# nichmorgan/better-search-rag-rust

Hardware: AMD Instinct MI355X
Metric: queries/sec + p50 latency, 768-d top-10 over N vectors @1/2/4/8 GPU (higher is better)
Workload: dtype f32; 1 GPU; configs[2]: 10M x 768 f32 corpus sharded over the N GPUs, 1000 batched queries, top-10; rows_total=10000000, rows_per_gpu_rank0=10000000, queries=1000, top_k=10, dim=768, parallelism=corpus sharded over 1 GPU(s) (interval_by_rank)

## Files before the change

better-search-rag-rust_amd/csrc/index.cpp:

```cpp
#include <math.h>
#include <stdio.h>
#include <string.h>

#include <algorithm>

#include "internal.hpp"
#include "kernels.hpp"

namespace bsr {

constexpr uint32_t kMaxKForFilter = 200;

static thread_local std::string g_err;

int set_error(int code, const char* fmt, ...) {
    char buf[1024];
    va_list ap;
    va_start(ap, fmt);
    vsnprintf(buf, sizeof buf, fmt, ap);
    va_end(ap);
    g_err = buf;
    return code;
}
void clear_error() { g_err.clear(); }
// ... 325 lines not shown
    if (nq > kSkinnyMaxQ || ix->n < kSkinnyTopMinRows || kp_for(k) > 63 || k > 64 || ix->op_row_bytes > 16 * 64 ||
        ix->ld % 64 != 0 || ix->ld > 1024 || !rescore_kp_enabled())
        return 0;
    const uint32_t slots = 4 * skinny_top_lists((uint32_t)ix->n);
    return slots <= 64u * kTopKeysPerLane ? slots : 0;
}

static int filter_buffers(bsr_index* ix, uint32_t nq, uint32_t qpad, uint32_t k, uint32_t cap_in = 0) {
    const uint32_t kp = kp_for(k);
    const uint32_t cap = std::max(cap_in ? cap_in : cap_for(k), top_slots(ix, nq, k));
    ix->stats.n_candidates = kp;
    BSR_TRY(ix->tau.ensure((size_t)qpad * sizeof(float)));
    BSR_TRY(ix->cand.ensure((size_t)qpad * cap * sizeof(uint64_t)));
    BSR_TRY(ix->cnt.ensure(((size_t)qpad + 8 * kTailCounters + kGangWords) * sizeof(uint32_t)));
    BSR_TRY(ix->cand_rows.ensure((size_t)nq * kp * sizeof(uint32_t)));
    BSR_TRY(ix->ncand.ensure((size_t)nq * sizeof(uint32_t)));
    BSR_TRY(ix->tau_excl.ensure((size_t)nq * sizeof(float)));
    BSR_TRY(ix->fail.ensure((size_t)nq * sizeof(uint32_t)));
    BSR_TRY(ix->fail2.ensure((size_t)nq * sizeof(uint32_t)));
    return BSR_OK;
}

static GemmArgs gemm_args(bsr_index* ix, uint32_t qpad) {
    GemmArgs g{};
    g.A = ix->fop.as<uint8_t>();
    g.B = ix->qop.as<uint8_t>();
    g.row_bytes = ix->op_row_bytes;
    g.n_qt = qpad / kFilterTile;
    g.a_scale = ix->ascale.as<float>();
    g.b_scale = ix->qscale.as<float>();
    return g;
}

static int sample_pass(bsr_index* ix, uint32_t nq, uint32_t qpad, uint32_t k, uint64_t* smax, uint32_t ks_in,
                       uint32_t cap_in) {
    BSR_TRY(filter_buffers(ix, nq, qpad, k, cap_in));
    const bool skinny = nq <= kSkinnyMaxQ;
    const uint32_t cap = cap_in ? cap_in : cap_for(k);
    const uint32_t ks = ks_in ? ks_in : ks_for(k);
    const uint32_t BM = kFilterTile;
    const uint64_t n = ix->n;
    GemmArgs g = gemm_args(ix, qpad);
    uint32_t* status = ix->d_status;
    if (n > cap) {
        const uint32_t n_s = (uint32_t)((n + kSampleStride - 1) / kSampleStride);
        const uint32_t n_rt_s = (n_s + BM - 1) / BM;
        const bool compact = n_s >= 32u * 8u * ks;
        const uint32_t s_ld = compact ? n_rt_s * (BM / 32) : n_rt_s * BM;
        const uint32_t n_vals = compact ? (n_s + 31) / 32 : n_s;
        BSR_TRY(ix->S.ensure((size_t)qpad * s_ld * sizeof(float)));
        g.A = ix->fop_s.as<uint8_t>();
        g.a_stride = ix->op_row_bytes;
        g.a_scale = ix->ascale_s.as<float>();
        g.a_scale_rows = kSampleScaleRows;
        g.n_rows = n_s;
        g.n_rt = n_rt_s;
        g.S = ix->S.as<float>();
        g.s_ld = s_ld;
        g.s_compact = compact ? 1u : 0u;
        BSR_HIP(launch_timed(ix, ix->ev_sample, [&](hipEvent_t e0, hipEvent_t e1) {
            return skinny ? launch_filter_skinny_sample(g, ix->stream, e0, e1)
                          : launch_filter_sample(g, ix->stream, e0, e1);
        }, 2));
        BSR_HIP(launch_select_tau(ix->S.as<float>(), s_ld, n_vals, nq, qpad, ix->qflags.as<uint32_t>(), ks,
                                  ix->tau.as<float>(), ix->cnt.as<uint32_t>(), status, ix->stream, smax));
    } else {
        BSR_HIP(launch_select_tau(nullptr, 0, 0, nq, qpad, ix->qflags.as<uint32_t>(), ks, ix->tau.as<float>(),
                                  ix->cnt.as<uint32_t>(), status, ix->stream, smax));
    }
    return BSR_OK;
}

static int emit_pass(bsr_index* ix, uint32_t nq, uint32_t qpad, uint32_t k, uint32_t cap_in) {
    const bool skinny = nq <= kSkinnyMaxQ;
    const uint32_t BM = kFilterTile;
    const uint64_t n = ix->n;
    GemmArgs g = gemm_args(ix, qpad);
    g.a_stride = ix->op_row_bytes;
    g.a_scale_rows = kQuantBlock;
    g.n_rows = (uint32_t)n;
    g.n_rt = (uint32_t)((n + BM - 1) / BM);
    g.tau = ix->tau.as<float>();
    g.cand = ix->cand.as<uint64_t>();
    g.cnt = ix->cnt.as<uint32_t>();
    g.cap = cap_in ? cap_in : cap_for(k);
    g.tail = g.n_qt <= kTailCounters ? ix->cnt.as<uint32_t>() + qpad : nullptr;
    BSR_HIP(launch_timed(ix, ix->ev_emit, [&](hipEvent_t e0, hipEvent_t e1) {
        return skinny ? launch_filter_skinny_emit(g, ix->stream, e0, e1)
                      : launch_filter_emit(g, ix->stream, e0, e1);
    }));
    return BSR_OK;
}

static uint32_t top_layout_lab() {
    const char* lay = getenv("BSR_TOP_LAYOUT");
    return lay && lay[0] == '0' ? 0u : 2u;
}

static int top_pass(bsr_index* ix, uint32_t nq, uint32_t qpad, uint32_t k) {
    BSR_TRY(filter_buffers(ix, nq, qpad, k));
    GemmArgs g = gemm_args(ix, qpad);
    g.a_stride = ix->op_row_bytes;
    g.a_scale_rows = kQuantBlock;
    g.n_rows = (uint32_t)ix->n;
    g.n_rt = (uint32_t)((ix->n + kFilterTile - 1) / kFilterTile);
    g.cand = ix->cand.as<uint64_t>();
    g.cnt = ix->cnt.as<uint32_t>();
    g.cap = top_slots(ix, nq, k);
    g.status = ix->d_status;
    g.n_q = nq;
    g.top_layout = top_layout_lab();
    BSR_HIP(launch_timed(ix, ix->ev_emit, [&](hipEvent_t e0, hipEvent_t e1) {
        return launch_filter_skinny_top(g, ix->stream, e0, e1);
    }));
    return BSR_OK;
}

static int run_filter(bsr_index* ix, uint32_t nq, uint32_t qpad, uint32_t k, uint32_t* next_status, bool publish) {
    const uint32_t top = top_slots(ix, nq, k);
    if (top) {
        BSR_TRY(top_pass(ix, nq, qpad, k));
    } else {
// ... 170 lines not shown
    qa.qf32 = qf32.as<float>();
    qa.nb = nb.as<float>();
    qa.qop = qop.p;
    qa.qscale = qscale.as<float>();
    qa.ebound = ebound.as<float>();
    qa.qflags = qflags.as<uint32_t>();
    qa.qids = qids_id.as<int32_t>();
    qa.status = d_status;
    qa.with_op = use_filter;
    const bool publish = use_filter && n > 0 && (!profiling(ix) || prof_level <= 1);
    auto enqueue_search = [&]() -> int {
        BSR_HIP(launch_query_prep(qa, stream));
        if (n == 0) {
            BSR_HIP(hipMemsetAsync(keys.p, 0xff, (size_t)nq * k * sizeof(uint64_t), stream));
        } else if (!use_filter) {
            stats.n_exact_direct = nq;
            BSR_TRY(run_exact_scan(ix, qids_id.as<int32_t>(), nq, k));
        } else {
            BSR_TRY(run_filter(ix, nq, qpad, k, next_status, publish));
        }
        if (!(use_filter && n > 0))
            BSR_HIP(launch_finalize(keys.as<uint64_t>(), nq, k, n, global_offset, d_idx, d_dist, d_cnt, next_status,
                                    nullptr, d_status, stream));
        ev_end(ix, ev_total);
        if (!publish) BSR_HIP(hipMemcpyAsync(h_res, res[cur].p, res_bytes, hipMemcpyDeviceToHost, stream));
        return BSR_OK;
    };
    if (publish) __atomic_store_n(h_flag, 0u, __ATOMIC_RELEASE);

    const bool top = use_filter && top_slots(ix, nq, k) != 0;
    if (top) stats.search_path |= BSR_PATH_SKINNY_TOP;
    const bool graphable = use_filter && n > 0 && (!profiling(ix) || prof_level == 0) && !force_threshold;
    SearchGraph& gs = graphs[cur];
    const uint32_t lay = (top ? top_layout_lab() : 2u) | (skinny_glds_on() ? 0x100u : 0u);
    const bool same_shape = warm.nq == nq && warm.k == k && warm.qsrc == qsrc && warm.n == n &&
                            warm.timed == (profiling(ix) ? prof_level : 0) && warm.top == top &&
                            warm.top_layout == lay;
    const int timed_level = profiling(ix) ? prof_level : 0;
    if (graphable && gs.exec && gs.nq == nq && gs.k == k && gs.qsrc == qsrc && gs.n == n && gs.gen == g_alloc_gen &&
        gs.timed == timed_level && gs.top == top && gs.top_layout == lay) {
        BSR_HIP(hipGraphLaunch(gs.exec, stream));
        stats.n_candidates = kp_for(k);
        ++graph_replays;
        stats.graph_replay = 1;
    } else if (graphable && same_shape && warm.gen == g_alloc_gen) {
        if (gs.exec) { (void)hipGraphExecDestroy(gs.exec); gs.exec = nullptr; }
        BSR_HIP(hipStreamBeginCapture(stream, hipStreamCaptureModeThreadLocal));
        const uint64_t gen0 = g_alloc_gen;
        capturing = true;
        const int rc = enqueue_search();
        capturing = false;
        hipGraph_t graph = nullptr;
        const hipError_t ec = hipStreamEndCapture(stream, &graph);
        if (rc != BSR_OK) { if (graph) (void)hipGraphDestroy(graph); return rc; }
        if (ec != hipSuccess || g_alloc_gen != gen0) {
            if (graph) (void)hipGraphDestroy(graph);
            return set_error(BSR_E_HIP, "search graph capture failed: %s", hipGetErrorString(ec));
        }
        hipGraphExec_t exec = nullptr;
        const hipError_t ei = hipGraphInstantiate(&exec, graph, nullptr, nullptr, 0);
        (void)hipGraphDestroy(graph);
        if (ei != hipSuccess) return set_error(BSR_E_HIP, "hipGraphInstantiate: %s", hipGetErrorString(ei));
        gs = SearchGraph{exec, nq, k, qsrc, n, g_alloc_gen, timed_level, top, lay};
        BSR_HIP(hipGraphLaunch(gs.exec, stream));
        ++graph_replays;
        stats.graph_replay = 1;
    } else {
// ... 288 lines not shown
        stats.search_path |= BSR_PATH_MASK_LIST;
        BSR_TRY(build_list());
        BSR_TRY(run_list_scan(ix, qids.as<int32_t>(), nfail, k, A));
        BSR_TRY(finalize_and_read());
    }
    return BSR_OK;
}

bool bsr_index::gtau_eligible(uint32_t nq, uint32_t k) const {
    return loaded && nq > 0 && k >= 1 && k <= cfg.max_k && k <= kMaxKForFilter && approx_ok && n > cap_for(k);
}

int bsr_index::gtau_prepare(const float* queries, uint32_t nq, uint32_t k) {
    if (!gtau_eligible(nq, k)) return set_error(BSR_E_STATE, "global-threshold search not applicable");
    if (!queries) return set_error(BSR_E_INVALID, "null queries");
    BSR_HIP(hipSetDevice(device));
    stats = bsr_search_stats{};
    stats.n_queries = nq;
    stats.row_ebound = row_ebound;
    BSR_TRY(prepare_result(nq, k));
    const uint32_t qpad = (uint32_t)round_up(nq, kFilterTile);
    const uint32_t ks = ks_for(k);
    BSR_TRY(qf32.ensure((size_t)qpad * ld * sizeof(float)));
    BSR_TRY(nb.ensure((size_t)qpad * sizeof(float)));
    BSR_TRY(qop.ensure((size_t)qpad * op_row_bytes));
    BSR_TRY(qscale.ensure((size_t)qpad * sizeof(float)));
    BSR_TRY(ebound.ensure((size_t)qpad * sizeof(float)));
    BSR_TRY(qflags.ensure((size_t)qpad * sizeof(uint32_t)));
    BSR_TRY(qids_id.ensure((size_t)qpad * sizeof(int32_t)));
    BSR_TRY(keys.ensure((size_t)nq * k * sizeof(uint64_t)));
    BSR_TRY(smax.ensure((size_t)qpad * ks * sizeof(uint64_t)));
    if (!is_device_ptr(queries)) BSR_TRY(q_in.ensure((size_t)nq * dim * sizeof(float)));
    BSR_TRY(filter_buffers(this, nq, qpad, k));
    const uint32_t n_s = (uint32_t)((n + kSampleStride - 1) / kSampleStride);
    const uint32_t n_rt_s = (n_s + kFilterTile - 1) / kFilterTile;
    const bool compact = n_s >= 32u * 8u * ks;
    const uint32_t s_ld = compact ? n_rt_s * (kFilterTile / 32) : n_rt_s * kFilterTile;
    BSR_TRY(S.ensure((size_t)qpad * s_ld * sizeof(float)));
    gt_nq = nq;
    gt_k = k;
    gt_qpad = qpad;
    gt_ks = ks;
    return BSR_OK;
}

int bsr_index::gtau_phase_a(const float* queries, int part) {
    bsr_index* ix = this;
    const uint32_t nq = gt_nq, k = gt_k, qpad = gt_qpad;
    if (part == 1) {
        BSR_TRY(sample_pass(ix, nq, qpad, k, smax.as<uint64_t>()));
        return BSR_OK;
    }
    const float* qsrc = queries;
    if (!is_device_ptr(queries)) {
        BSR_HIP(hipMemcpyAsync(q_in.p, queries, (size_t)nq * dim * sizeof(float), hipMemcpyHostToDevice, stream));
        qsrc = q_in.as<float>();
    }
    ev_begin(ix, ev_total);
    QueryPrepArgs qa{};
    qa.q = qsrc;
    qa.nq = nq;
    qa.qpad = qpad;
    qa.dim = dim;
    qa.ld = ld;
    qa.ea_max = flags.as<uint32_t>() + 1;
    qa.qf32 = qf32.as<float>();
    qa.nb = nb.as<float>();
    qa.qop = qop.p;
    qa.qscale = qscale.as<float>();
    qa.ebound = ebound.as<float>();
    qa.qflags = qflags.as<uint32_t>();
// ... 105 lines not shown
```

better-search-rag-rust_amd/csrc/internal.hpp:

```cpp
#pragma once

#include <hip/hip_runtime.h>
#include <stdarg.h>
#include <stdint.h>

#include <atomic>

#include <string>
#include <vector>

#include "bsr.h"
#include "kernels.hpp"

namespace bsr {

int set_error(int code, const char* fmt, ...);
void clear_error();

#define BSR_HIP(call)                                                                       \
    do {                                                                                    \
        hipError_t e_ = (call);                                                             \
        if (e_ != hipSuccess)                                                               \
            return ::bsr::set_error(BSR_E_HIP, "%s failed: %s (%s:%d)", #call,              \
                                    hipGetErrorString(e_), __FILE__, __LINE__);             \
// ... 20 lines not shown
void* coherent_host_alias(const void* p);
hipError_t stream_wait(hipStream_t s);
hipError_t flag_wait(const uint32_t* flag, hipStream_t s);
int select_device(int device);

static inline uint64_t round_up(uint64_t x, uint64_t m) { return (x + m - 1) / m * m; }

struct Events {
    hipEvent_t a = nullptr, b = nullptr;
    bool armed = false;
    ~Events();
    int create();
};

}

struct bsr_index {
    bsr_config cfg{};
    int device = 0;
    hipStream_t stream = nullptr;
    uint32_t dim = 0, ld = 0;
    uint64_t n = 0, n_pad = 0, global_offset = 0;
    bool loaded = false;
    bool approx_ok = false;
    uint32_t row_flags = 0;
    uint32_t op_row_bytes = 0;
    float row_ebound = 0.0f;

    bsr::DevBuf rows;
    bsr::DevBuf na;
    bsr::DevBuf fop;
    bsr::DevBuf fop_s;
    bsr::DevBuf ascale_s;
    bsr::DevBuf ascale;
    bsr::DevBuf flags;

    bsr::DevBuf q_in, qf32, nb, qop, qscale, ebound, qflags, tau, S, cand, cnt, cand_rows, ncand,
        tau_excl, keys, fail, fail2, part, qids, qids_id, tmp;

    bsr::DevBuf res[2];
    uint8_t* h_res = nullptr;
    uint8_t* h_res_dev = nullptr;
    size_t h_res_bytes = 0;
    uint32_t* h_flag = nullptr;
    uint32_t* h_flag_dev = nullptr;
    bsr::DevBuf pub_ticket;
    uint32_t cur = 0;
    bool next_status_clean = false;
    size_t res_off_cnt = 0, res_off_dist = 0, res_off_idx = 0, res_off_x = 0, res_bytes = 0;
    uint32_t* d_status = nullptr;
    uint32_t* d_cnt = nullptr;
    float* d_dist = nullptr;
    uint64_t* d_idx = nullptr;
    float* d_x = nullptr;

    std::vector<uint32_t> h_qflags, h_fail;

    bsr_search_stats stats{};
    bsr_profile prof{};
    bsr::Events ev_emit, ev_sample, ev_select, ev_rescore, ev_scan, ev_total;
    int prof_level = 2;

    struct SearchGraph {
        hipGraphExec_t exec = nullptr;
        uint32_t nq = 0, k = 0;
        const float* qsrc = nullptr;
// ... 31 lines not shown
```

better-search-rag-rust_amd/csrc/k_filter.hip:

```cpp
#include <cstdlib>
#include "bsr_device.hpp"
#include "kernels.hpp"

#include <hip/hip_ext.h>

#include <math.h>

#include <algorithm>
#include <type_traits>
#include <utility>

namespace bsr {

typedef __attribute__((ext_vector_type(4))) int i32x4_t;
typedef __attribute__((ext_vector_type(16))) int i32x16_t;
typedef __attribute__((address_space(3))) void lds_void_t;

struct OpI8 {
    using frag_t = i32x4_t;
    using acc_t = i32x16_t;
    static constexpr bool kInt = true;
    __device__ __forceinline__ static acc_t mfma(const frag_t& a, const frag_t& b, const acc_t& c) {
        return __builtin_amdgcn_mfma_i32_32x32x32_i8(a, b, c, 0, 0, 0);
    }
};

constexpr int kSlots = 4;
constexpr int kSliceB = 64;
constexpr int kWCap = 256;
constexpr int kThreads = 512;

__device__ __forceinline__ void wait_vm0() { asm volatile("s_waitcnt vmcnt(0)" ::: "memory"); }

template <int N>
__device__ __forceinline__ void mid_barrier() {
    if constexpr (N == 8) asm volatile("s_waitcnt vmcnt(8) lgkmcnt(0)\n\ts_barrier" ::: "memory");
    else if constexpr (N == 6) asm volatile("s_waitcnt vmcnt(6) lgkmcnt(0)\n\ts_barrier" ::: "memory");
    else if constexpr (N == 4) asm volatile("s_waitcnt vmcnt(4) lgkmcnt(0)\n\ts_barrier" ::: "memory");
// ... 375 lines not shown
    do {                                                                                \
        __builtin_amdgcn_sched_barrier(0);                                              \
        asm volatile("s_memtime %0\n\ts_waitcnt lgkmcnt(0)" : "=s"(V_)::"memory");       \
        __builtin_amdgcn_sched_barrier(0);                                              \
    } while (0)
#endif
template <bool EMIT, int NK, int EPI = 0, int TAILX = 8, int GANG = 2, int RING = 0, int L2 = 0, int FW = 1,
          int KSB = 0>
__global__ __launch_bounds__(512, 1) void k_filter_qs16(GemmArgs p) {
    constexpr bool DEFER = EPI == 1, STAGE = EPI == 2 && EMIT;
    constexpr bool SPLIT = EPI == 3 && EMIT;
    constexpr int S = RING ? 12 : 8, A = RING == 1 ? 9 : RING == 2 ? 10 : 6;
    constexpr int kWaitN = A - 4, kYoung = A - 4, kClaimUse = ((A - 4) % 2 == 0 ? A - 3 : A - 2) + 1;
    constexpr int BM = 128, BN = kFilterTile, NT = 512, SLOT = BM * kSliceB;
    constexpr int CAP = RING ? 7 : 10;
    static_assert(NK % 2 == 0 && NK >= 2 && NK <= 12, "even slice counts up to 768 bytes");
    constexpr int QCAP = 32, NSTG = 16;
    constexpr int ST_QL = 0, ST_STG = ST_QL + BN * QCAP * 8, ST_META = ST_STG + NSTG * 1024,
                  ST_QPAR = ST_META + NSTG * 16, ST_QCNT = ST_QPAR + BN * 8, ST_CNT = ST_QCNT + BN * 4,
                  ST_BYTES = ST_CNT + 16;
    constexpr int EM_BYTES = !EMIT ? 0 : STAGE ? ST_BYTES : NT * 2 * CAP * 8;
    constexpr int SB_BYTES = EMIT ? 0 : kSampleTilesPerWG * 4 * BN * 4;
    __shared__ __attribute__((aligned(1024))) uint8_t lds[S * SLOT + EM_BYTES + SB_BYTES + 16];
    float* const sbuf = reinterpret_cast<float*>(lds + S * SLOT + EM_BYTES);
    uint32_t* const lds_ids = reinterpret_cast<uint32_t*>(lds + S * SLOT + EM_BYTES + SB_BYTES);
    const int tid = threadIdx.x, lane = tid & 63, w = tid >> 6;
    const uint32_t wu = __builtin_amdgcn_readfirstlane(tid >> 6);
    const bool dfr = DEFER || (SPLIT && wu >= 4);
    uint64_t* const lkeys = reinterpret_cast<uint64_t*>(lds + S * SLOT) + tid;
    uint32_t ecnt[2] = {0, 0};

    const uint32_t b = blockIdx.x, xcd = b & 7, slot = b >> 3;
    const uint32_t G = (gridDim.x >> 3) / p.n_qt;
    const uint32_t n_rt = (p.n_rows + BM - 1) / BM;
    const bool active = slot < G * p.n_qt;
    const uint32_t qt = active ? slot % p.n_qt : 0;
#ifdef BSR_FILTER_COUNTERS
    const uint32_t g0 = (xcd ^ g_lab_xcd_xor) * G + (active ? slot / p.n_qt : 0);
#else
    const uint32_t g0 = xcd * G + (active ? slot / p.n_qt : 0);
#endif
    const uint32_t RG = 8 * G;
    const uint32_t my_rt = (active && g0 < n_rt) ? (n_rt - 1 - g0) / RG + 1 : 0;
    const uint32_t J = my_rt * NK;
    constexpr uint32_t kEnd = 0xFFFFFFFFu;
    constexpr bool kStaticSched = NK > A;
    const bool dyn = EMIT && kStaticSched && p.tail != nullptr && active;
    const uint32_t n_st = dyn ? n_rt - n_rt / (TAILX ? TAILX : kTailDiv) : n_rt;
    const uint32_t my_static = (active && g0 < n_st) ? (n_st - 1 - g0) / RG + 1 : 0;
    const uint32_t n_tail = n_rt - n_st, pool_sz = (n_tail + 7) / 8;
    uint32_t cpool = xcd, pools_tried = 1;
    auto pool_n = [&](uint32_t x) -> uint32_t {
        const uint32_t lo = x * pool_sz;
        return lo >= n_tail ? 0u : min(pool_sz, n_tail - lo);
    };
    auto claim_raw = [&]() -> uint32_t {
        uint32_t z;
        asm volatile("v_mov_b32 %0, 0" : "=v"(z));
        return atomicAdd(p.tail + (TAILX ? cpool * p.n_qt : 0u) + qt + z, 1u);
    };
    auto tail_id = [&](uint32_t v) -> uint32_t {
        if constexpr (!TAILX) {
            return n_st + v < n_rt ? n_st + v : kEnd;
        } else {
            for (;;) {
                if (v < pool_n(cpool)) return n_st + cpool * pool_sz + v;
                if (pools_tried == 8) return kEnd;
// ... 59 lines not shown
            asm volatile("ds_add_rtn_u32 %0, %1, %2\n\ts_waitcnt lgkmcnt(0)" : "=v"(pos) : "v"(addr), "v"(1u) : "memory");
            if (pos < (uint32_t)QCAP) {
                st_ql[ql * QCAP + pos] = score_key(v, row);
            } else {
                const uint32_t q = qt * BN + ql;
                const uint32_t gp = atomicAdd(p.cnt + q, 1u);
                if (gp < p.cap) p.cand[(uint64_t)q * p.cap + gp] = score_key(v, row);
                __builtin_amdgcn_s_waitcnt(0x0F70);
            }
        }
    };
    auto st_process = [&](uint32_t n) {
        for (uint32_t v = tid; v < n * 256; v += NT) {
            const uint32_t e = v >> 8, i = v & 255, l = i >> 2;
            const int iv = st_blk[v];
            const uint32_t* m = st_meta + 4 * e;
            st_append(iv, __uint_as_float(m[2]), m[0] + 4 * (l >> 4) + (i & 3), m[1] + (l & 15));
        }
    };
    if constexpr (STAGE) {
        if (lane < 16)
#pragma unroll
            for (int nb = 0; nb < 2; ++nb) {
                const uint32_t ql = w * 32 + nb * 16 + lane;
                st_qpar[2 * ql] = sbq[nb];
                st_qpar[2 * ql + 1] = tau[nb];
            }
        if (tid < BN) st_qcnt[tid] = 0;
        if (tid == 0) *st_cnt = 0;
    }

    const uint32_t lrow = w * 16 + (lane >> 2);
    const uint32_t lchunk = ((lane & 3) ^ qs16_swz(lrow)) * 16;
    auto tile_src_rt = [&](uint32_t rt, __amdgpu_buffer_rsrc_t& rs, uint32_t& off) {
        rs = __builtin_amdgcn_make_buffer_rsrc((void*)(p.A + (uint64_t)rt * BM * p.a_stride), 0,
                                               BM * (uint32_t)p.a_stride, 0x00020000);
        const uint32_t r = (EMIT || rt * BM + lrow < p.n_rows) ? lrow : p.n_rows - 1 - rt * BM;
        off = r * (uint32_t)p.a_stride + lchunk;
    };
    auto tile_src = [&](uint32_t ti, __amdgpu_buffer_rsrc_t& rs, uint32_t& off) { tile_src_rt(g0 + ti * RG, rs, off); };
    constexpr bool kStatic = kStaticSched;
    __amdgpu_buffer_rsrc_t rs_cur, rs_nxt;
    uint32_t off_cur = 0, off_nxt = 0;
    auto dma_static = [&](uint32_t jj, int kt) {
        uint8_t* la = lds + (jj % S) * SLOT + wu * 1024;
        if (kt + A < NK)
            __builtin_amdgcn_raw_ptr_buffer_load_lds(rs_cur, (lds_void_t*)la, 16, off_cur, (kt + A) * kSliceB, 0, 0);
        else
            __builtin_amdgcn_raw_ptr_buffer_load_lds(rs_nxt, (lds_void_t*)la, 16, off_nxt, (kt + A - NK) * kSliceB, 0, 0);
    };
    uint32_t iss_ti = 0, iss_kt = 0, aoff_dma = 0;
    __amdgpu_buffer_rsrc_t rsrc_a;
    auto issue_dma = [&](uint32_t jj) {
        uint8_t* la = lds + (jj % S) * SLOT + wu * 1024;
        __builtin_amdgcn_raw_ptr_buffer_load_lds(rsrc_a, (lds_void_t*)la, 16, aoff_dma, iss_kt * kSliceB, 0, 0);
        if (++iss_kt == NK) {
            iss_kt = 0;
            ++iss_ti;
            if (iss_ti < my_rt) tile_src(iss_ti, rsrc_a, aoff_dma);
        }
    };
    const uint32_t aoff0 = (lane & 15) * kSliceB + (((lane >> 4) ^ qs16_swz(lane & 15)) * 16);
    i32x4v_t fa[4];
    auto read_frag = [&](uint32_t jj, int rb) {
        fa[rb & 3] = *reinterpret_cast<const i32x4v_t*>(lds + (jj % S) * SLOT + rb * 1024 + aoff0);
    };

// ... 47 lines not shown
        nxt_id = g0 + RG;
    }
    const bool any_tile = cur_id != kEnd;
    const uint32_t pre = (dyn ? any_tile : J != 0) ? (uint32_t)A : 0u;
    if (any_tile) {
        tile_src_rt(cur_id, rsrc_a, aoff_dma);
        rs_cur = rsrc_a;
        off_cur = aoff_dma;
        tile_src_rt(nxt_id != kEnd ? nxt_id : cur_id, rs_nxt, off_nxt);
    }
    if (kStatic) {
        for (uint32_t jj = 0; jj < pre; ++jj) {
            uint8_t* la = lds + (jj % S) * SLOT + wu * 1024;
            __builtin_amdgcn_raw_ptr_buffer_load_lds(rs_cur, (lds_void_t*)la, 16, off_cur, jj * kSliceB, 0, 0);
        }
    } else {
        for (uint32_t jj = 0; jj < pre; ++jj) issue_dma(jj);
    }
    qs_barrier(pre >= 3 ? pre - 3 : 0);
    if (any_tile)
#pragma unroll
        for (int rb = 0; rb < 4; ++rb) read_frag(0, rb);

#ifdef BSR_FILTER_COUNTERS
    unsigned long long fcnt[5] = {0, 0, 0, 0, 0};
    if (EMIT && tid == 0 && blockIdx.x < 4096) g_filter_wg_stamps[blockIdx.x * 9] = __builtin_amdgcn_s_memrealtime();
#endif
#ifdef BSR_FILTER_STAMPS
    unsigned long long fst[8] = {0, 0, 0, 0, 0, 0, 0, 0}, st_a, st_b, st_loop0;
    BSR_FST(st_loop0);
#endif
    uint32_t t = 0;
    for (; cur_id != kEnd; ++t) {
        const uint32_t rt = cur_id;
        BSR_FCNT(4);
        if (kStatic && t) {
            rs_cur = rs_nxt;
            off_cur = off_nxt;
            tile_src_rt(nxt_id != kEnd ? nxt_id : cur_id, rs_nxt, off_nxt);
        }
        float4 scv = make_float4(1.0f, 1.0f, 1.0f, 1.0f);
        if (EMIT) scv = *reinterpret_cast<const float4*>(p.a_scale + (uint64_t)rt * (BM / kQuantBlock));
        uint32_t n2 = (t + 2 < my_static) ? g0 + (t + 2) * RG : kEnd;
        const bool req = dyn && t + 2 >= my_static && nxt_id != kEnd;
        uint32_t claimed = 0;
        if (req && tid == 0) claimed = claim_raw();
        const bool thr = gang && t + 2 < my_static;
        unsigned long long gold = 0;
        if (thr && tid == 0) gold = gang_raw();
        const int w0_req = ((req || thr) && w == 0) ? 1 : 0;
        float sc_tile = 1.0f;
        if constexpr (!EMIT) sc_tile = p.a_scale[rt * BM / kSampleScaleRows];
        static_for(std::make_integer_sequence<int, NK>{}, [&](auto KT) {
            constexpr int kt = decltype(KT)::value;
            const uint32_t jj = t * NK + kt;
            const bool bar_slice = (kt & 1) == 1;
#pragma unroll
            for (int rb = 0; rb < 8; ++rb) {
                if constexpr ((DEFER || SPLIT) && EMIT && kt == 0) {
                    if (dfr && (rb & 1) == 0 && t > 0) epi_pair(rb >> 1, sc_prev[rb >> 1], rt_prev);
                    asm volatile("" : "+v"(fa[rb & 3]));
                    __builtin_amdgcn_sched_barrier(0);
                }
#pragma unroll
                for (int nb = 0; nb < 2; ++nb) {
                    if (kt == 0) {
                        const i32x4v_t z = {};
                        acc[rb][nb] = __builtin_amdgcn_mfma_i32_16x16x64_i8(fa[rb & 3], fb[nb][kt], z, 0, 0, 0);
                    } else {
                        acc[rb][nb] = __builtin_amdgcn_mfma_i32_16x16x64_i8(fa[rb & 3], fb[nb][kt], acc[rb][nb], 0, 0, 0);
                    }
                }
                __builtin_amdgcn_sched_barrier(0);
                if (KSB && (rb & 1)) {
                } else if (rb < 4) {
                    read_frag(jj, rb + 4);
                } else {
                    read_frag(jj + 1, rb - 4);
                }
                if (kt == kClaimUse && rb == 0 && req && tid == 0) lds_ids[t & 1] = tail_id(claimed);
                if (GANG && kt == kClaimUse && rb == 0 && thr && tid == 0) gang_throttle(gold);
                if (bar_slice ? rb == 6 : rb == 1) {
                    if (kStatic) dma_static(jj + A, kt);
                    else issue_dma(jj + A);
                }
// ... 5 lines not shown
                        BSR_FST(st_b);
                        fst[6] += st_b - st_a;
                        st_a = st_b;
                        asm volatile("s_barrier" ::: "memory");
                        BSR_FST(st_b);
                        fst[kt == 1 ? 3 : 4] += st_b - st_a;
                    } else
#endif
                    qs_wait_n(kWaitN + ((EMIT && kt <= kYoung) ? 1 + w0_req : 0));
                }
                if constexpr (STAGE) {
                    if (kt == 1 && rb == 5) n_stg = min(*st_cnt, (uint32_t)NSTG);
                    if (kt == 2 && rb == 0 && n_stg) st_process(n_stg);
                    if (kt == 3 && rb == 5 && tid == 0) {
                        *st_cnt = 0;
                        asm volatile("s_waitcnt lgkmcnt(0)" ::: "memory");
                    }
                }
                __builtin_amdgcn_sched_barrier(0);
            }
        });
        if constexpr (KSB == 2 && EMIT) {
            i32x4v_t* xs = reinterpret_cast<i32x4v_t*>(lds + S * SLOT + (w % 5) * 16384) + lane;
#pragma unroll
            for (int i = 0; i < 16; ++i) xs[i * 64] = acc[i >> 1][i & 1];
            asm volatile("s_waitcnt lgkmcnt(0)" ::: "memory");
#pragma unroll
            for (int i = 0; i < 16; ++i) acc[i >> 1][i & 1] += xs[(15 - i) * 64];
        }
        const float sc[4] = {scv.x, scv.y, scv.z, scv.w};
        bool stored = false;
        if constexpr (!EMIT) {
            if (p.s_compact) {
#pragma unroll
                for (int g = 0; g < 4; ++g)
#pragma unroll
                    for (int nb = 0; nb < 2; ++nb) {
                        const i32x4v_t& x = acc[2 * g][nb];
                        const i32x4v_t& y = acc[2 * g + 1][nb];
                        int m = max(max(max(x[0], x[1]), max(x[2], x[3])), max(max(y[0], y[1]), max(y[2], y[3])));
                        const auto p16 = __builtin_amdgcn_permlane16_swap(m, m, false, false);
                        m = max((int)p16[0], (int)p16[1]);
                        const auto p32 = __builtin_amdgcn_permlane32_swap(m, m, false, false);
                        m = max((int)p32[0], (int)p32[1]);
                        const float v = ((float)m * sc_tile) * sbq[nb];
                        if (lane < 16) sbuf[((t % kSampleTilesPerWG) * 4 + g) * BN + (qq[nb] - qt * BN)] = v;
                    }
                if (t % kSampleTilesPerWG == kSampleTilesPerWG - 1 || t + 1 == my_rt) {
                    __syncthreads();
                    const uint32_t t0 = t - t % kSampleTilesPerWG, nt = t + 1 - t0;
                    for (uint32_t i = tid; i < nt * BN; i += NT) {
                        const uint32_t tt = i / BN, ql = i % BN;
                        const float4 v = make_float4(sbuf[(tt * 4 + 0) * BN + ql], sbuf[(tt * 4 + 1) * BN + ql],
                                                     sbuf[(tt * 4 + 2) * BN + ql], sbuf[(tt * 4 + 3) * BN + ql]);
                        *reinterpret_cast<float4*>(p.S + (uint64_t)(qt * BN + ql) * p.s_ld + (g0 + (t0 + tt) * RG) * 4) = v;
                    }
                    stored = true;
                }
            } else {
#pragma unroll
                for (int rb = 0; rb < 8; ++rb) {
                    const uint32_t rbase = rt * BM + rb * 16 + 4 * (lane >> 4);
#pragma unroll
                    for (int nb = 0; nb < 2; ++nb) {
                        const i32x4v_t& x = acc[rb][nb];
                        const float v0 = ((float)x[0] * sc_tile) * sbq[nb], v1 = ((float)x[1] * sc_tile) * sbq[nb];
                        const float v2 = ((float)x[2] * sc_tile) * sbq[nb], v3 = ((float)x[3] * sc_tile) * sbq[nb];
                        *reinterpret_cast<float4*>(p.S + (uint64_t)qq[nb] * p.s_ld + rbase) = make_float4(v0, v1, v2, v3);
                    }
                }
                stored = true;
            }
        } else if constexpr (STAGE) {
            const float sc_hi = fmaxf(fmaxf(sc[0], sc[1]), fmaxf(sc[2], sc[3]));
            const float sc_lo = fminf(fminf(sc[0], sc[1]), fminf(sc[2], sc[3]));
            int mrb[2];
            bool any = false;
#pragma unroll
// ... 142 lines not shown
            }
        }
    }
    if constexpr ((DEFER || SPLIT) && EMIT) {
        if (dfr && t > 0)
#pragma unroll
            for (int s = 0; s < 4; ++s) epi_pair(s, sc_prev[s], rt_prev);
    }
    wait_vm0();
#ifdef BSR_FILTER_STAMPS
    if (EMIT) {
        BSR_FST(st_b);
        fst[5] = st_b - st_loop0;
        if (lane == 0)
            for (int i = 0; i < 8; ++i) atomicAdd(&g_filter_stamps[i], fst[i]);
    }
#endif
    if constexpr (EMIT) {
        flush_ring(0);
        flush_ring(1);
#ifdef BSR_FILTER_COUNTERS
        if (lane == 0) {
            for (int i = 0; i < 4; ++i) atomicAdd(&g_filter_counters[i], fcnt[i]);
            if (blockIdx.x < 4096) g_filter_wg_stamps[blockIdx.x * 9 + 1 + w] = __builtin_amdgcn_s_memrealtime();
            if (blockIdx.x < 4096 && w == 0) {
                g_filter_wg_tiles[blockIdx.x * 2] = (unsigned int)fcnt[4];
                g_filter_wg_tiles[blockIdx.x * 2 + 1] = my_static;
            }
        }
#endif
    }
}


typedef __attribute__((ext_vector_type(4))) int i32x4_acc_t;

template <bool EMIT>
__global__ __launch_bounds__(256) void k_filter_skinny(GemmArgs p) {
    constexpr int KC = 8;
    const int lane = threadIdx.x & 63, w = threadIdx.x >> 6;
    const uint32_t q = lane & 15, h = lane >> 4;
    const uint32_t nk = p.row_bytes / kSliceB;
    const uint32_t n_groups = (p.n_rows + 31) / 32;
    const uint32_t nwaves = gridDim.x * 4;
    const float sbq = p.b_scale[q];
    const float tauq = EMIT ? p.tau[q] : 0.0f;
    const uint8_t* bq = p.B + (uint64_t)q * p.row_bytes + h * 16;
    for (uint32_t g = blockIdx.x * 4 + w; g < n_groups; g += nwaves) {
        uint32_t r0 = g * 32 + q, r1 = g * 32 + 16 + q;
        r0 = r0 < p.n_rows ? r0 : p.n_rows - 1;
        r1 = r1 < p.n_rows ? r1 : p.n_rows - 1;
        const uint8_t* a0 = p.A + (uint64_t)r0 * p.a_stride + h * 16;
        const uint8_t* a1 = p.A + (uint64_t)r1 * p.a_stride + h * 16;
        i32x4_acc_t acc0 = {0, 0, 0, 0}, acc1 = {0, 0, 0, 0};
        for (uint32_t s0 = 0; s0 < nk; s0 += KC) {
            i32x4_t fa0[KC], fa1[KC], fb[KC];
#pragma unroll
            for (int s = 0; s < KC; ++s) {
                if (s0 + s < nk) {
                    fa0[s] = *reinterpret_cast<const i32x4_t*>(a0 + (s0 + s) * kSliceB);
                    fa1[s] = *reinterpret_cast<const i32x4_t*>(a1 + (s0 + s) * kSliceB);
                    fb[s] = *reinterpret_cast<const i32x4_t*>(bq + (s0 + s) * kSliceB);
                }
            }
#pragma unroll
            for (int s = 0; s < KC; ++s) {
// ... 641 lines not shown
template <int MODE>
static void launch_skinny(const GemmArgs& a, hipStream_t s, hipEvent_t e0, hipEvent_t e1) {
    const uint32_t nk = a.row_bytes / kSliceB;
    if constexpr (MODE != kSkSample) {
        if (nk == 12 && skinny_glds_on()) {
            BSR_KLAUNCH((k_filter_skinny_glds<MODE, 12>), dim3(skinny2_grid(a.n_rows)), dim3(128), s, e0, e1, a);
            return;
        }
    }
    const dim3 g(nk <= 16 ? skinny2_grid(a.n_rows) : skinny_grid(a.n_rows)), b(256);
    if (nk <= 4) BSR_KLAUNCH((k_filter_skinny2<MODE, 4>), g, b, s, e0, e1, a);
    else if (nk <= 8) BSR_KLAUNCH((k_filter_skinny2<MODE, 8>), g, b, s, e0, e1, a);
    else if (nk <= 12) BSR_KLAUNCH((k_filter_skinny2<MODE, 12>), g, b, s, e0, e1, a);
    else if (nk <= 16) BSR_KLAUNCH((k_filter_skinny2<MODE, 16>), g, b, s, e0, e1, a);
    else if constexpr (MODE != kSkTop) BSR_KLAUNCH(k_filter_skinny<MODE == kSkEmit>, g, b, s, e0, e1, a);
}
hipError_t launch_filter_skinny_sample(const GemmArgs& a, hipStream_t s, hipEvent_t e0, hipEvent_t e1) {
    launch_skinny<kSkSample>(a, s, e0, e1);
    return hipGetLastError();
}
hipError_t launch_filter_skinny_emit(const GemmArgs& a, hipStream_t s, hipEvent_t e0, hipEvent_t e1) {
    launch_skinny<kSkEmit>(a, s, e0, e1);
    return hipGetLastError();
}
hipError_t launch_filter_skinny_top(const GemmArgs& a, hipStream_t s, hipEvent_t e0, hipEvent_t e1) {
    if (a.row_bytes / kSliceB > 16) return hipErrorInvalidValue;
    launch_skinny<kSkTop>(a, s, e0, e1);
    return hipGetLastError();
}

static bool gang_possible(const GemmArgs& a, uint32_t grid) {
    if (!a.tail || a.n_qt < 2 || a.n_qt > 4) return false;
    const uint32_t G = (grid / 8) / a.n_qt, RG = 8 * G;
    const uint32_t n_rt = (a.n_rows + 127) / 128, n_st = n_rt - n_rt / 8;
    return RG && n_st && (n_st - 1) / RG + 1 >= kGangMinTiles;
}

template <bool EMIT>
static void launch_filter(const GemmArgs& a, hipStream_t s, hipEvent_t e0, hipEvent_t e1) {
    const uint32_t nk = a.row_bytes / kSliceB, grid = filter_grid(a.n_qt);
    if (nk % 2 == 0 && nk <= 12) {
        const dim3 g(grid), b(512);
        if (EMIT && nk == 12 && !gang_possible(a, grid)) {
            BSR_KLAUNCH((k_filter_qs16<EMIT, 12, 0, 8, 0, 0, 1, 0>), g, b, s, e0, e1, a);
            return;
        }
        switch (nk) {
            case 2: BSR_KLAUNCH((k_filter_qs16<EMIT, 2>), g, b, s, e0, e1, a); return;
            case 4: BSR_KLAUNCH((k_filter_qs16<EMIT, 4>), g, b, s, e0, e1, a); return;
            case 6: BSR_KLAUNCH((k_filter_qs16<EMIT, 6>), g, b, s, e0, e1, a); return;
            case 8: BSR_KLAUNCH((k_filter_qs16<EMIT, 8>), g, b, s, e0, e1, a); return;
            case 10: BSR_KLAUNCH((k_filter_qs16<EMIT, 10>), g, b, s, e0, e1, a); return;
            default: BSR_KLAUNCH((k_filter_qs16<EMIT, 12>), g, b, s, e0, e1, a); return;
        }
    }
    BSR_KLAUNCH((k_filter<OpI8, EMIT>), dim3(grid), dim3(kThreads), s, e0, e1, a);
}
hipError_t launch_filter_sample(const GemmArgs& a, hipStream_t s, hipEvent_t e0, hipEvent_t e1) {
    launch_filter<false>(a, s, e0, e1);
    return hipGetLastError();
}
hipError_t launch_filter_emit(const GemmArgs& a, hipStream_t s, hipEvent_t e0, hipEvent_t e1) {
    launch_filter<true>(a, s, e0, e1);
    return hipGetLastError();
}
hipError_t launch_select_tau(const float* S, uint32_t s_ld, uint32_t n_s, uint32_t nq, uint32_t qpad,
                             const uint32_t* qflags, uint32_t ks, float* tau, uint32_t* cnt, uint32_t* status,
                             hipStream_t s, uint64_t* smax) {
    if (ks > 2 * kWave) return hipErrorInvalidValue;
    static const int m_on = [] {
        const char* v = getenv("BSR_SELECT_TAU_M");
        return v && v[0] == '0' ? 0 : v && v[0] == '2' ? 2 : 1;
    }();
    if (m_on && ks <= kWave && (qpad <= 16 || m_on == 2) && n_s > 32 * kWave && n_s <= 16 * 16 * kWave)
        hipLaunchKernelGGL(k_select_tau_m<16>, dim3(qpad), dim3(1024), 0, s, S, s_ld, n_s, nq, qpad, qflags, ks,
                           tau, cnt, status, smax);
    else if (ks <= kWave && n_s <= 32 * kWave && qpad % 4 == 0)
        hipLaunchKernelGGL(k_select_tau_w<32>, dim3(qpad / 4), dim3(256), 0, s, S, s_ld, n_s, nq, qpad, qflags, ks,
                           tau, cnt, status, smax);
    else if (ks > kWave)
        hipLaunchKernelGGL(k_select_tau<2>, dim3(qpad), dim3(256), 0, s, S, s_ld, n_s, nq, qpad, qflags, ks, tau,
                           cnt, status, smax);
    else
        hipLaunchKernelGGL(k_select_tau<1>, dim3(qpad), dim3(256), 0, s, S, s_ld, n_s, nq, qpad, qflags, ks, tau,
                           cnt, status, smax);
    return hipGetLastError();
}
hipError_t launch_global_tau(const uint64_t* g, uint32_t P, uint32_t qpad, uint32_t nq, uint32_t ks,
                             const uint32_t* qflags, float* tau, hipStream_t s) {
    if (ks > 2 * kWave || P == 0) return hipErrorInvalidValue;
    if (ks > kWave)
        hipLaunchKernelGGL(k_global_tau<2>, dim3(qpad / 4), dim3(256), 0, s, g, P, qpad, nq, ks, qflags, tau);
    else
        hipLaunchKernelGGL(k_global_tau<1>, dim3(qpad / 4), dim3(256), 0, s, g, P, qpad, nq, ks, qflags, tau);
    return hipGetLastError();
}
// ... 26 lines not shown
```

better-search-rag-rust_amd/csrc/kernels.hpp:

```cpp
#pragma once

#include <hip/hip_runtime.h>
#include <stdint.h>

namespace bsr {

constexpr uint32_t kLdAlign = 64;
constexpr uint32_t kRowPad = 256;
constexpr uint32_t kScanQF = 8;
constexpr uint32_t kSampleStride = 32;
constexpr uint32_t kQuantBlock = 32;
constexpr uint32_t kSampleScaleRows = 128;
constexpr uint32_t kFilterTile = 256;

constexpr uint32_t kRowNonFinite = 1u;
constexpr uint32_t kRowNormOvf = 2u;
constexpr uint32_t kRowNormRange = 4u;

constexpr uint32_t kQueryNonFinite = 1u;
constexpr uint32_t kQueryNoApprox = 2u;

enum StatusWord : uint32_t { kStFail = 0, kStEmitted = 1, kStQueryFlags = 2, kStFail2 = 3, kStWords = 4 };

hipError_t launch_synth_uniform(float* out, uint64_t row0, uint64_t n_rows, uint32_t dim,
// ... 32 lines not shown

constexpr uint32_t kMaskBlockWords = 256;
static inline uint32_t mask_blocks(uint64_t n) {
    const uint64_t words = (n + 63) / 64, b = (words + kMaskBlockWords - 1) / kMaskBlockWords;
    return (uint32_t)(b < 1 ? 1 : b);
}
hipError_t launch_mask_list_count(const uint64_t* allow, uint64_t n, uint32_t* blk, hipStream_t s);
hipError_t launch_mask_list_scatter(const uint64_t* allow, uint64_t n, const uint32_t* blk, uint32_t n_list,
                                    uint32_t* list, hipStream_t s);
hipError_t launch_mask_cut(uint64_t* cand, uint32_t* cnt, uint32_t cap, uint32_t nq, const uint64_t* allow,
                           uint64_t n, uint32_t* raw, uint32_t* items, hipStream_t s);

struct GemmArgs {
    const uint8_t* A;
    uint64_t a_stride;
    uint32_t n_rows;
    uint32_t a_scale_rows;
    const uint8_t* B;
    uint32_t row_bytes;
    uint32_t n_rt, n_qt;
    const float* a_scale;
    const float* b_scale;
    float* S;
    uint32_t s_ld;
    uint32_t s_compact;
    const float* tau;
    uint64_t* cand;
    uint32_t* cnt;
    uint32_t cap;
    uint32_t* tail;
    uint32_t* status;
    uint32_t n_q;
    uint32_t top_layout;
};
constexpr uint32_t kTailDiv = 8;
constexpr uint32_t kTailCounters = 64;
constexpr uint32_t kGangWords = 2 * 256;
constexpr uint32_t kGangMinTiles = 600;
hipError_t launch_filter_sample(const GemmArgs& a, hipStream_t s, hipEvent_t e0 = nullptr,
                                hipEvent_t e1 = nullptr);
hipError_t launch_filter_emit(const GemmArgs& a, hipStream_t s, hipEvent_t e0 = nullptr,
                              hipEvent_t e1 = nullptr);
constexpr uint32_t kSkinnyMaxQ = 16;
hipError_t launch_filter_skinny_sample(const GemmArgs& a, hipStream_t s, hipEvent_t e0 = nullptr, hipEvent_t e1 = nullptr);
hipError_t launch_filter_skinny_emit(const GemmArgs& a, hipStream_t s, hipEvent_t e0 = nullptr, hipEvent_t e1 = nullptr);
hipError_t launch_filter_skinny_top(const GemmArgs& a, hipStream_t s, hipEvent_t e0 = nullptr, hipEvent_t e1 = nullptr);
uint32_t skinny_top_lists(uint32_t n_rows);
bool skinny_glds_on();
constexpr uint64_t kSkinnyTopMinRows = 2u << 20;

hipError_t launch_select_tau(const float* S, uint32_t s_ld, uint32_t n_s, uint32_t nq,
                             uint32_t qpad, const uint32_t* qflags, uint32_t ks, float* tau,
                             uint32_t* cnt, uint32_t* status, hipStream_t s, uint64_t* smax = nullptr);
hipError_t launch_global_tau(const uint64_t* g, uint32_t P, uint32_t qpad, uint32_t nq, uint32_t ks,
                             const uint32_t* qflags, float* tau, hipStream_t s);
hipError_t launch_select_cand(const uint64_t* cand, const uint32_t* cnt, uint32_t cap,
                              uint32_t nq, const float* tau, uint32_t kp, uint32_t* cand_rows,
                              uint32_t* ncand, float* tau_excl, hipStream_t s);

struct RescoreArgs {
    const float* rows;
    uint32_t ld, dim;
    const float* na;
    const float* qf32;
    const float* nb;
    uint32_t n_items;
    const uint32_t* n_items_dev;
    const uint32_t* qlist;
    const uint32_t* cand_rows;
    const uint32_t* ncand;
    uint32_t kp;
    const float* tau_excl;
    const uint64_t* cand_keys;
    const uint32_t* cnt;
    uint32_t cap;
// ... 92 lines not shown
```

Baseline: 170,200 queries/s.

## Sample whole corpus tiles in place and skip them in emit with fixup

The sampling pass now scores every 32nd full 128-row tile of the real quantized corpus, using per-block scales, instead of a separate strided sample copy. The emit pass skips those tiles, so no rows are scored twice. A new fixup kernel rescans only the sampled 32-row blocks whose max reaches tau and emits their candidates. This removes the redundant sample GEMM work but adds an extra kernel launch and changes the tau statistics, which are now drawn from contiguous blocks rather than strided rows.

```diff
diff --git a/better-search-rag-rust_amd/csrc/index.cpp b/better-search-rag-rust_amd/csrc/index.cpp
--- a/better-search-rag-rust_amd/csrc/index.cpp
+++ b/better-search-rag-rust_amd/csrc/index.cpp
@@ -381,32 +381,71 @@
     return g;
 }
 
+struct SampleLayout {
+    uint32_t n_s, n_rt_s;
+    bool compact;
+    uint32_t tiles;
+    uint32_t s_ld, n_vals;
+};
+static bool sample_tiles_on() {
+    const char* v = getenv("BSR_SAMPLE_TILES");
+    return !(v && v[0] == '0');
+}
+static SampleLayout sample_layout(const bsr_index* ix, uint32_t nq, uint32_t ks) {
+    SampleLayout L{};
+    const uint32_t BM = kFilterTile;
+    L.n_s = (uint32_t)((ix->n + kSampleStride - 1) / kSampleStride);
+    L.n_rt_s = (L.n_s + BM - 1) / BM;
+    L.compact = L.n_s >= 32u * 8u * ks;
+    const uint32_t nk = ix->op_row_bytes / 64;
+    const bool qs16 = ix->op_row_bytes % 64 == 0 && nk % 2 == 0 && nk >= 2 && nk <= 12;
+    if (L.compact && nq > kSkinnyMaxQ && qs16 && sample_tiles_on()) L.tiles = sample_tiles_for(ix->n);
+    if (L.tiles) {
+        const uint64_t last0 = ((uint64_t)(L.tiles - 1) * kSampleTileEvery + kSampleTilePhase) * 128;
+        const uint64_t valid = std::min<uint64_t>(128, ix->n - last0);
+        L.s_ld = 4 * L.tiles;
+        L.n_vals = 4 * (L.tiles - 1) + (uint32_t)((valid + kQuantBlock - 1) / kQuantBlock);
+    } else {
+        L.s_ld = L.compact ? L.n_rt_s * (BM / 32) : L.n_rt_s * BM;
+        L.n_vals = L.compact ? (L.n_s + 31) / 32 : L.n_s;
+    }
+    return L;
+}
+
 static int sample_pass(bsr_index* ix, uint32_t nq, uint32_t qpad, uint32_t k, uint64_t* smax, uint32_t ks_in,
                        uint32_t cap_in) {
     BSR_TRY(filter_buffers(ix, nq, qpad, k, cap_in));
+    ix->smp_tiles = 0;
     const bool skinny = nq <= kSkinnyMaxQ;
     const uint32_t cap = cap_in ? cap_in : cap_for(k);
     const uint32_t ks = ks_in ? ks_in : ks_for(k);
-    const uint32_t BM = kFilterTile;
     const uint64_t n = ix->n;
     GemmArgs g = gemm_args(ix, qpad);
     uint32_t* status = ix->d_status;
     if (n > cap) {
-        const uint32_t n_s = (uint32_t)((n + kSampleStride - 1) / kSampleStride);
-        const uint32_t n_rt_s = (n_s + BM - 1) / BM;
-        const bool compact = n_s >= 32u * 8u * ks;
-        const uint32_t s_ld = compact ? n_rt_s * (BM / 32) : n_rt_s * BM;
-        const uint32_t n_vals = compact ? (n_s + 31) / 32 : n_s;
+        const SampleLayout L = sample_layout(ix, nq, ks);
+        const uint32_t s_ld = L.s_ld, n_vals = L.n_vals;
         BSR_TRY(ix->S.ensure((size_t)qpad * s_ld * sizeof(float)));
-        g.A = ix->fop_s.as<uint8_t>();
         g.a_stride = ix->op_row_bytes;
-        g.a_scale = ix->ascale_s.as<float>();
-        g.a_scale_rows = kSampleScaleRows;
-        g.n_rows = n_s;
-        g.n_rt = n_rt_s;
+        if (L.tiles) {
+            g.a_scale_rows = kQuantBlock;
+            g.n_rows = (uint32_t)n;
+            g.n_rt = L.tiles;
+            g.s_tiles = L.tiles;
+            g.s_vals = n_vals;
+            ix->smp_tiles = L.tiles;
+            ix->smp_ld = s_ld;
+            ix->smp_vals = n_vals;
+        } else {
+            g.A = ix->fop_s.as<uint8_t>();
+            g.a_scale = ix->ascale_s.as<float>();
+            g.a_scale_rows = kSampleScaleRows;
+            g.n_rows = L.n_s;
+            g.n_rt = L.n_rt_s;
+        }
         g.S = ix->S.as<float>();
         g.s_ld = s_ld;
-        g.s_compact = compact ? 1u : 0u;
+        g.s_compact = L.compact ? 1u : 0u;
         BSR_HIP(launch_timed(ix, ix->ev_sample, [&](hipEvent_t e0, hipEvent_t e1) {
             return skinny ? launch_filter_skinny_sample(g, ix->stream, e0, e1)
                           : launch_filter_sample(g, ix->stream, e0, e1);
@@ -434,9 +473,16 @@
     g.cnt = ix->cnt.as<uint32_t>();
     g.cap = cap_in ? cap_in : cap_for(k);
     g.tail = g.n_qt <= kTailCounters ? ix->cnt.as<uint32_t>() + qpad : nullptr;
+    g.s_tiles = skinny ? 0u : ix->smp_tiles;
+    g.S = ix->S.as<float>();
+    g.s_ld = ix->smp_ld;
+    g.s_vals = ix->smp_vals;
+    g.n_q = nq;
     BSR_HIP(launch_timed(ix, ix->ev_emit, [&](hipEvent_t e0, hipEvent_t e1) {
-        return skinny ? launch_filter_skinny_emit(g, ix->stream, e0, e1)
-                      : launch_filter_emit(g, ix->stream, e0, e1);
+        hipError_t r = skinny ? launch_filter_skinny_emit(g, ix->stream, e0, e1)
+                              : launch_filter_emit(g, ix->stream, e0, e1);
+        if (r == hipSuccess && g.s_tiles) r = launch_sample_fixup(g, ix->stream);
+        return r;
     }));
     return BSR_OK;
 }
@@ -673,7 +719,8 @@
     if (top) stats.search_path |= BSR_PATH_SKINNY_TOP;
     const bool graphable = use_filter && n > 0 && (!profiling(ix) || prof_level == 0) && !force_threshold;
     SearchGraph& gs = graphs[cur];
-    const uint32_t lay = (top ? top_layout_lab() : 2u) | (skinny_glds_on() ? 0x100u : 0u);
+    const uint32_t lay = (top ? top_layout_lab() : 2u) | (skinny_glds_on() ? 0x100u : 0u) |
+                         (sample_tiles_on() ? 0x200u : 0u);
     const bool same_shape = warm.nq == nq && warm.k == k && warm.qsrc == qsrc && warm.n == n &&
                             warm.timed == (profiling(ix) ? prof_level : 0) && warm.top == top &&
                             warm.top_layout == lay;
@@ -1028,11 +1075,7 @@
     BSR_TRY(smax.ensure((size_t)qpad * ks * sizeof(uint64_t)));
     if (!is_device_ptr(queries)) BSR_TRY(q_in.ensure((size_t)nq * dim * sizeof(float)));
     BSR_TRY(filter_buffers(this, nq, qpad, k));
-    const uint32_t n_s = (uint32_t)((n + kSampleStride - 1) / kSampleStride);
-    const uint32_t n_rt_s = (n_s + kFilterTile - 1) / kFilterTile;
-    const bool compact = n_s >= 32u * 8u * ks;
-    const uint32_t s_ld = compact ? n_rt_s * (kFilterTile / 32) : n_rt_s * kFilterTile;
-    BSR_TRY(S.ensure((size_t)qpad * s_ld * sizeof(float)));
+    BSR_TRY(S.ensure((size_t)qpad * sample_layout(this, nq, ks).s_ld * sizeof(float)));
     gt_nq = nq;
     gt_k = k;
     gt_qpad = qpad;
diff --git a/better-search-rag-rust_amd/csrc/internal.hpp b/better-search-rag-rust_amd/csrc/internal.hpp
--- a/better-search-rag-rust_amd/csrc/internal.hpp
+++ b/better-search-rag-rust_amd/csrc/internal.hpp
@@ -76,6 +76,7 @@
     bsr::DevBuf fop;
     bsr::DevBuf fop_s;
     bsr::DevBuf ascale_s;
+    uint32_t smp_tiles = 0, smp_ld = 0, smp_vals = 0;
     bsr::DevBuf ascale;
     bsr::DevBuf flags;
 
diff --git a/better-search-rag-rust_amd/csrc/k_filter.hip b/better-search-rag-rust_amd/csrc/k_filter.hip
--- a/better-search-rag-rust_amd/csrc/k_filter.hip
+++ b/better-search-rag-rust_amd/csrc/k_filter.hip
@@ -4,6 +4,7 @@
 
 #include <hip/hip_ext.h>
 
+#include <limits.h>
 #include <math.h>
 
 #include <algorithm>
@@ -445,7 +446,12 @@
 
     const uint32_t b = blockIdx.x, xcd = b & 7, slot = b >> 3;
     const uint32_t G = (gridDim.x >> 3) / p.n_qt;
-    const uint32_t n_rt = (p.n_rows + BM - 1) / BM;
+    const uint32_t n_phys = (p.n_rows + BM - 1) / BM;
+    const uint32_t n_rt = !p.s_tiles ? n_phys : EMIT ? n_phys - p.s_tiles : p.s_tiles;
+    auto phys = [&](uint32_t lt) -> uint32_t {
+        if (!p.s_tiles) return lt;
+        return EMIT ? lt + lt / (kSampleTileEvery - 1) : lt * kSampleTileEvery + kSampleTilePhase;
+    };
     const bool active = slot < G * p.n_qt;
     const uint32_t qt = active ? slot % p.n_qt : 0;
 #ifdef BSR_FILTER_COUNTERS
@@ -571,7 +577,8 @@
 
     const uint32_t lrow = w * 16 + (lane >> 2);
     const uint32_t lchunk = ((lane & 3) ^ qs16_swz(lrow)) * 16;
-    auto tile_src_rt = [&](uint32_t rt, __amdgpu_buffer_rsrc_t& rs, uint32_t& off) {
+    auto tile_src_rt = [&](uint32_t lt, __amdgpu_buffer_rsrc_t& rs, uint32_t& off) {
+        const uint32_t rt = phys(lt);
         rs = __builtin_amdgcn_make_buffer_rsrc((void*)(p.A + (uint64_t)rt * BM * p.a_stride), 0,
                                                BM * (uint32_t)p.a_stride, 0x00020000);
         const uint32_t r = (EMIT || rt * BM + lrow < p.n_rows) ? lrow : p.n_rows - 1 - rt * BM;
@@ -685,7 +692,7 @@
 #endif
     uint32_t t = 0;
     for (; cur_id != kEnd; ++t) {
-        const uint32_t rt = cur_id;
+        const uint32_t rt = phys(cur_id);
         BSR_FCNT(4);
         if (kStatic && t) {
             rs_cur = rs_nxt;
@@ -702,8 +709,17 @@
         unsigned long long gold = 0;
         if (thr && tid == 0) gold = gang_raw();
         const int w0_req = ((req || thr) && w == 0) ? 1 : 0;
-        float sc_tile = 1.0f;
-        if constexpr (!EMIT) sc_tile = p.a_scale[rt * BM / kSampleScaleRows];
+        float sc_tile = 1.0f, sc_blk[4] = {1.0f, 1.0f, 1.0f, 1.0f};
+        if constexpr (!EMIT) {
+            if (p.s_tiles) {
+#pragma unroll
+                for (int g = 0; g < 4; ++g) sc_blk[g] = p.a_scale[rt * (BM / kQuantBlock) + g];
+            } else {
+                sc_tile = p.a_scale[rt * BM / kSampleScaleRows];
+#pragma unroll
+                for (int g = 0; g < 4; ++g) sc_blk[g] = sc_tile;
+            }
+        }
         static_for(std::make_integer_sequence<int, NK>{}, [&](auto KT) {
             constexpr int kt = decltype(KT)::value;
             const uint32_t jj = t * NK + kt;
@@ -775,18 +791,26 @@
         bool stored = false;
         if constexpr (!EMIT) {
             if (p.s_compact) {
+                const bool part = p.s_tiles && rt * BM + BM > p.n_rows;
 #pragma unroll
                 for (int g = 0; g < 4; ++g)
 #pragma unroll
                     for (int nb = 0; nb < 2; ++nb) {
-                        const i32x4v_t& x = acc[2 * g][nb];
-                        const i32x4v_t& y = acc[2 * g + 1][nb];
+                        i32x4v_t x = acc[2 * g][nb], y = acc[2 * g + 1][nb];
+                        if (part) {
+                            const uint32_t r0 = rt * BM + g * 32 + 4 * (lane >> 4);
+#pragma unroll
+                            for (int r = 0; r < 4; ++r) {
+                                x[r] = r0 + r < p.n_rows ? x[r] : INT_MIN;
+                                y[r] = r0 + 16 + r < p.n_rows ? y[r] : INT_MIN;
+                            }
+                        }
                         int m = max(max(max(x[0], x[1]), max(x[2], x[3])), max(max(y[0], y[1]), max(y[2], y[3])));
                         const auto p16 = __builtin_amdgcn_permlane16_swap(m, m, false, false);
                         m = max((int)p16[0], (int)p16[1]);
                         const auto p32 = __builtin_amdgcn_permlane32_swap(m, m, false, false);
                         m = max((int)p32[0], (int)p32[1]);
-                        const float v = ((float)m * sc_tile) * sbq[nb];
+                        const float v = ((float)m * sc_blk[g]) * sbq[nb];
                         if (lane < 16) sbuf[((t % kSampleTilesPerWG) * 4 + g) * BN + (qq[nb] - qt * BN)] = v;
                     }
                 if (t % kSampleTilesPerWG == kSampleTilesPerWG - 1 || t + 1 == my_rt) {
@@ -995,6 +1019,76 @@
     }
 }
 
+
+__global__ __launch_bounds__(256) void k_sample_fixup(GemmArgs p) {
+    constexpr int NKM = 12, U = 4;
+    const uint32_t q = blockIdx.x;
+    const float tq = p.tau[q];
+    if (!(tq < INFINITY)) return;
+    const int tid = threadIdx.x, lane = tid & 63;
+    const uint32_t w0 = __builtin_amdgcn_readfirstlane(tid >> 6) * 64;
+    const uint32_t c = lane & 3, rr = lane >> 2;
+    const int nk = p.row_bytes / kSliceB;
+    const float sbq = p.b_scale[q];
+    i32x4_t fb[NKM];
+#pragma unroll
+    for (int s = 0; s < NKM; ++s)
+        fb[s] = s < nk ? *reinterpret_cast<const i32x4_t*>(p.B + (uint64_t)q * p.row_bytes + s * kSliceB + c * 16)
+                       : i32x4_t{0, 0, 0, 0};
+    auto block = [&](uint32_t j) {
+        const uint32_t r0 = ((j >> 2) * kSampleTileEvery + kSampleTilePhase) * 128 + (j & 3) * 32;
+        const float sc = p.a_scale[r0 / kQuantBlock];
+        i32x4_t fa[2][NKM];
+#pragma unroll
+        for (int h = 0; h < 2; ++h) {
+            const uint8_t* a = p.A + (uint64_t)(r0 + 16 * h + rr) * p.a_stride + c * 16;
+#pragma unroll
+            for (int s = 0; s < NKM; ++s)
+                if (s < nk) fa[h][s] = *reinterpret_cast<const i32x4_t*>(a + s * kSliceB);
+        }
+#pragma unroll
+        for (int h = 0; h < 2; ++h) {
+            int acc = 0;
+#pragma unroll
+            for (int s = 0; s < NKM; ++s)
+                if (s < nk)
+#pragma unroll
+                    for (int e = 0; e < 4; ++e) acc = __builtin_amdgcn_sdot4(fa[h][s][e], fb[s][e], acc, false);
+            acc += (int)xor_lane32<1>((uint32_t)acc);
+            acc += (int)xor_lane32<2>((uint32_t)acc);
+            const float v = ((float)acc * sc) * sbq;
+            const uint32_t row = r0 + 16 * h + rr;
+            const bool pass = c == 0 && v >= tq && row < p.n_rows;
+            const uint64_t mk = __ballot(pass);
+            if (mk) {
+                uint32_t gp = 0;
+                if (lane == 0) gp = atomicAdd(p.cnt + q, (uint32_t)__builtin_popcountll(mk));
+                gp = __builtin_amdgcn_readfirstlane(gp);
+                const uint32_t pos = gp + (uint32_t)__builtin_popcountll(mk & ((1ull << lane) - 1ull));
+                if (pass && pos < p.cap) p.cand[(uint64_t)q * p.cap + pos] = score_key(v, row);
+            }
+        }
+    };
+    const float* srow = p.S + (uint64_t)q * p.s_ld;
+    for (uint32_t base = 0; base < p.s_vals; base += U * 256) {
+        float sv[U];
+#pragma unroll
+        for (int u = 0; u < U; ++u) {
+            const uint32_t j = base + u * 256 + tid;
+            sv[u] = j < p.s_vals ? srow[j] : -INFINITY;
+        }
+#pragma unroll
+        for (int u = 0; u < U; ++u) {
+            const uint32_t j = base + u * 256 + tid;
+            uint64_t m = __ballot(j < p.s_vals && sv[u] >= tq);
+            while (m) {
+                const uint32_t b = (uint32_t)__builtin_ctzll(m);
+                m &= m - 1;
+                block(base + u * 256 + w0 + b);
+            }
+        }
+    }
+}
 
 typedef __attribute__((ext_vector_type(4))) int i32x4_acc_t;
 
@@ -1702,7 +1796,7 @@
 static bool gang_possible(const GemmArgs& a, uint32_t grid) {
     if (!a.tail || a.n_qt < 2 || a.n_qt > 4) return false;
     const uint32_t G = (grid / 8) / a.n_qt, RG = 8 * G;
-    const uint32_t n_rt = (a.n_rows + 127) / 128, n_st = n_rt - n_rt / 8;
+    const uint32_t n_rt = (a.n_rows + 127) / 128 - a.s_tiles, n_st = n_rt - n_rt / 8;
     return RG && n_st && (n_st - 1) / RG + 1 >= kGangMinTiles;
 }
 
@@ -1732,6 +1826,12 @@
 }
 hipError_t launch_filter_emit(const GemmArgs& a, hipStream_t s, hipEvent_t e0, hipEvent_t e1) {
     launch_filter<true>(a, s, e0, e1);
+    return hipGetLastError();
+}
+hipError_t launch_sample_fixup(const GemmArgs& a, hipStream_t s) {
+    const uint32_t nk = a.row_bytes / kSliceB;
+    if (!a.s_tiles || !a.n_q || nk < 1 || nk > 12 || a.row_bytes % kSliceB) return hipErrorInvalidValue;
+    hipLaunchKernelGGL(k_sample_fixup, dim3(a.n_q), dim3(256), 0, s, a);
     return hipGetLastError();
 }
 hipError_t launch_select_tau(const float* S, uint32_t s_ld, uint32_t n_s, uint32_t nq, uint32_t qpad,
diff --git a/better-search-rag-rust_amd/csrc/kernels.hpp b/better-search-rag-rust_amd/csrc/kernels.hpp
--- a/better-search-rag-rust_amd/csrc/kernels.hpp
+++ b/better-search-rag-rust_amd/csrc/kernels.hpp
@@ -88,7 +88,11 @@
     uint32_t* status;
     uint32_t n_q;
     uint32_t top_layout;
-};
+    uint32_t s_tiles, s_vals;
+};
+constexpr uint32_t kSampleTileEvery = 32;
+constexpr uint32_t kSampleTilePhase = 31;
+static inline uint32_t sample_tiles_for(uint64_t n) { return (uint32_t)(((n + 127) / 128) / kSampleTileEvery); }
 constexpr uint32_t kTailDiv = 8;
 constexpr uint32_t kTailCounters = 64;
 constexpr uint32_t kGangWords = 2 * 256;
@@ -97,6 +101,7 @@
                                 hipEvent_t e1 = nullptr);
 hipError_t launch_filter_emit(const GemmArgs& a, hipStream_t s, hipEvent_t e0 = nullptr,
                               hipEvent_t e1 = nullptr);
+hipError_t launch_sample_fixup(const GemmArgs& a, hipStream_t s);
 constexpr uint32_t kSkinnyMaxQ = 16;
 hipError_t launch_filter_skinny_sample(const GemmArgs& a, hipStream_t s, hipEvent_t e0 = nullptr, hipEvent_t e1 = nullptr);
 hipError_t launch_filter_skinny_emit(const GemmArgs& a, hipStream_t s, hipEvent_t e0 = nullptr, hipEvent_t e1 = nullptr);
```

Result: faster. 173,800 queries/s, median of 6 (+2.1%).
